# leggedrobotics/delora

Measured on AMD Instinct MI355X. Metric: training scan-pairs/sec, KITTI 64x2048 range images, higher is better.
Workload: dtype f32; 1 GPU; KITTI-shaped 64x2048, batch=8 pairs/GPU, raw scans of ~141k points (ragged, raster order), steps rotate over 8 distinct HBM-resident batches, online normals, ResNet pose CNN (11.9M params, identity-pretrained state), Adam; BASELINE configs[1]; global_batch=8, parallelism=dp1, cnn=fp32, cnn_impl=hip trunk: fp32 MFMA, fused Winograd F(2x2,3x3) + direct implicit GEMM, channels_last=False, hip_graph=False, distinct_batches=8, priming_steps=8

## Files before the change

delora_amd/csrc/conv.hip:

```cpp
#include <type_traits>

#include "common.h"
#include "conv_geom.h"
#include "wgrad_batch.h"

typedef float f32x16 __attribute__((ext_vector_type(16)));
typedef float f32x4 __attribute__((ext_vector_type(4)));

__device__ __forceinline__ __amdgpu_buffer_rsrc_t cv_rsrc(const float* base, unsigned bytes) {
  return __builtin_amdgcn_make_buffer_rsrc(const_cast<float*>(base), 0, (int)bytes, 0x00020000);
}
__device__ __forceinline__ f32x4 cv_ld16(__amdgpu_buffer_rsrc_t rs, unsigned voff, unsigned soff) {
  return __builtin_bit_cast(f32x4, __builtin_amdgcn_raw_buffer_load_b128(rs, (int)voff, (int)soff, 0));
}
#define CV_ZERO_OFF 0x80000000u

#define CV_THREADS 256
#define CV_EPI_ADD 1u
#define CV_EPI_ACT 2u
#define CV_EPI_DACT 4u
#define CV_EPI_ADD_GRID 8u
#define CV_ACT_NONE 0
#define CV_ACT_TANH 1
#define CV_ACT_RELU 2
// ... 4 lines not shown
  float* y;
  const float* add;
  const float* dsrc;
  int N, H, W, C, K, Ho, Wo;
  int act;
  unsigned epi;
  int Hout, Wout;
  int wrap;
  const float* seam;
};

__device__ __forceinline__ float cv_act(float v, int act) {
  if (act == CV_ACT_TANH) return dl_tanh(v);
  if (act == CV_ACT_RELU) return v < 0.f ? 0.f : v;
  return v;
}
__device__ __forceinline__ float cv_dact(float y, int act) {
  if (act == CV_ACT_TANH) return 1.f - y * y;
  if (act == CV_ACT_RELU) return y <= 0.f ? 0.f : 1.f;
  return 1.f;
}

__device__ __forceinline__ int cv_xcd_swizzle(int id, int n) {
  const int q = n / 8, r = n % 8, xcd = id % 8, k = id / 8;
  return (xcd < r ? xcd * (q + 1) : r * (q + 1) + (xcd - r) * q) + k;
}

template <int BM, int BN, int CK, int TW, class G, bool BT, int WGN>
#ifndef CV_MINWAVES
#define CV_MINWAVES 2
#endif
__global__ __launch_bounds__(CV_THREADS, CV_MINWAVES) void k_conv_f32(ConvArgs a) {
  constexpr int TH = BM / TW;
  constexpr int SH = G::ISH, SW = G::ISW;
  constexpr int RH = (TH - 1) * SH + G::EH, RW = (TW - 1) * SW + G::EW;
  constexpr int S = CK + 4;
  constexpr int TAPS = G::NT;
  constexpr int C4 = CK / 4;
  constexpr int IN_FLOATS = RH * RW * S;
  constexpr int W_FLOATS = BT ? TAPS * CK * BN : TAPS * BN * S;
  constexpr int NI = RH * RW * C4;
  constexpr int NW = BT ? CK * TAPS * (BN / 4) : BN * TAPS * C4;
  constexpr int NI_IT = (NI + CV_THREADS - 1) / CV_THREADS, NW_IT = (NW + CV_THREADS - 1) / CV_THREADS;
  constexpr int WGM = 4 / WGN;
  constexpr int WM = BM / 32 / WGM, WN = BN / 32 / WGN;
  static_assert(BM % TW == 0 && BM % (32 * WGM) == 0 && BN % (32 * WGN) == 0 && CK % 8 == 0, "tile shape");
  static_assert(TAPS > 0, "a stride phase without taps has no launch");
  static_assert((S / 4) % 2 == 1, "pixel stride must be 4*odd floats");
  constexpr int EPW = WN * 32, ES = EPW + 4;
  constexpr int LDS_HOLD = (BM == 256 && TW == 128 && CK == 8 && BT) ? 160 * 1024 / 3 / 4 + 16 : 0;
  constexpr int LDS_USED = IN_FLOATS + W_FLOATS > 4 * 32 * ES ? IN_FLOATS + W_FLOATS : 4 * 32 * ES;
  constexpr int LDS_FLOATS = LDS_USED > LDS_HOLD ? LDS_USED : LDS_HOLD;
  __shared__ __attribute__((aligned(16))) float lds[LDS_FLOATS];
  float* in_lds = lds;
  float* w_lds = lds + IN_FLOATS;

  const int tid = threadIdx.x, lane = tid & 63, wave = tid >> 6;
  const int li = lane & 31, half = lane >> 5;
  const int wm = wave / WGN, wn = wave % WGN;
  const int KT = a.K / BN;
  const int tiles_w = (a.Wo + TW - 1) / TW, tiles_h = (a.Ho + TH - 1) / TH;
  const int ntiles = a.N * tiles_h * tiles_w * KT;
  const int t = cv_xcd_swizzle(blockIdx.x, ntiles);
  const int kt = t % KT;
  int pt = t / KT;
  const int tw_i = pt % tiles_w; pt /= tiles_w;
  const int th_i = pt % tiles_h;
  const int n = pt / tiles_h;
  const int ho0 = th_i * TH, wo0 = tw_i * TW, k0 = kt * BN;
  const int h_base = ho0 * SH + G::H0, w_base = wo0 * SW + G::W0;
  const float* xn = a.x + (size_t)n * a.H * a.W * a.C;

  const unsigned x_bytes = (unsigned)(a.H * a.W * a.C) * 4u, w_bytes = (unsigned)(a.K * a.C * G::WTAPS) * 4u;
  const __amdgpu_buffer_rsrc_t x_rs = cv_rsrc(xn, x_bytes), w_rs = cv_rsrc(a.w, w_bytes);
  const unsigned x_zero = CV_ZERO_OFF;
  unsigned in_g[NI_IT];
  int in_l[NI_IT];
#pragma unroll
  for (int it = 0; it < NI_IT; ++it) {
    const int q = min(tid + it * CV_THREADS, NI - 1);
    const int c4 = q % C4, pc = q / C4;
    const int col = pc % RW, row = pc / RW;
    const int h = h_base + row;
    int w = w_base + col;
    const bool col_in = w >= 0 && w < a.W;
    w = w < 0 ? w + a.W : w;
    w = w >= a.W ? w - a.W : w;
    in_l[it] = pc * S + c4 * 4;
    in_g[it] = (h >= 0 && h < a.H && (a.wrap ? w < a.W : col_in)) ? (unsigned)((h * a.W + w) * a.C + c4 * 4) * 4u : x_zero;
  }
  unsigned w_g[NW_IT];
  int w_l[NW_IT];
#pragma unroll
  for (int it = 0; it < NW_IT; ++it) {
    const int q = min(tid + it * CV_THREADS, NW - 1);
    if (!BT) {
      const int c4 = q % C4, t2 = q / C4;
      const int tap = t2 % TAPS, kk = t2 / TAPS;
      w_g[it] = (unsigned)(((k0 + kk) * G::WTAPS + G::wt(tap)) * a.C + c4 * 4) * 4u;
      w_l[it] = (tap * BN + kk) * S + c4 * 4;
    } else {
      const int co4 = q % (BN / 4), t2 = q / (BN / 4);
      const int tap = t2 % TAPS, kr = t2 / TAPS;
      w_g[it] = (unsigned)((kr * G::WTAPS + G::wt(tap)) * a.K + k0 + co4 * 4) * 4u;
      w_l[it] = (tap * CK + kr) * BN + co4 * 4;
    }
  }

  f32x16 acc[WM][WN];
#pragma unroll
  for (int i = 0; i < WM; ++i)
#pragma unroll
    for (int j = 0; j < WN; ++j)
#pragma unroll
      for (int r = 0; r < 16; ++r) acc[i][j][r] = 0.f;

  int a_off[WM];
// ... 371 lines not shown
};
__global__ __launch_bounds__(CV_THREADS) void k_wgrad_reduce_batch(WgReduceBatchArgs b) {
  const int l = dl_table_slot<DL_WGRAD_BATCH>(b.first_block, b.n, (int)blockIdx.x);
  dl_slab_sum_body(b.part[l], b.nslabs[l], b.count[l], b.dw[l], ((size_t)((int)blockIdx.x - b.first_block[l]) * CV_THREADS + threadIdx.x) * 4);
}
__global__ __launch_bounds__(CV_THREADS) void k_wgrad_reduce(const float* __restrict__ part, int nslabs, size_t count,
                                                             float* __restrict__ dw) {
  dl_slab_sum_body(part, nslabs, count, dw, ((size_t)blockIdx.x * CV_THREADS + threadIdx.x) * 4);
}


template <int BM, int BN, int CK, int TW, class G, bool BT, int WGN>
static int launch_conv(const ConvArgs& a, hipStream_t st) {
  constexpr int TH = BM / TW;
  if (a.K % BN || a.C % CK) return 1;
  const int ntiles = a.N * ((a.Ho + TH - 1) / TH) * ((a.Wo + TW - 1) / TW) * (a.K / BN);
  const double px_ = (double)a.N * a.Ho * a.Wo;
  constexpr int ks_ = G::WTAPS == 9 ? 3 : 1;
  const DlProfTag tag{"k_conv_f32", BT ? "dgrad" : "fwd", a.N, a.H, a.W, a.C, a.K, ks_, BT ? G::OSH : G::ISH, BT ? G::OSW : G::ISW, 2.0 * px_ * a.K * a.C * G::NT,
                      4.0 * ((double)a.N * a.H * a.W * a.C + px_ * a.K + (double)G::WTAPS * a.K * a.C)};
  DL_LAUNCH(tag, (k_conv_f32<BM, BN, CK, TW, G, BT, WGN>), dim3(ntiles), dim3(CV_THREADS), st, a);
  return 0;
}

#ifndef CV_BN
#define CV_BN 64
#endif
#ifndef CV_CK
#define CV_CK 16
#endif
#ifndef CV_WGN
#define CV_WGN 2
#endif

#ifdef CV_TUNE
int g_cv_variant = 0;
template <class G, bool BT, int BM, int BN, int CKK, int WGNN>
static int variant_conv(const ConvArgs& a, hipStream_t st) {
  if (a.Wo % 128 == 0 && !launch_conv<BM, BN, CKK, 128, G, BT, WGNN>(a, st)) return 0;
  if (a.Wo % 64 == 0 && !launch_conv<BM, BN, CKK, 64, G, BT, WGNN>(a, st)) return 0;
  return 1;
}
#endif

static int cv_pick_tw(int Ho, int Wo, int bm, int min_tw) {
  int best = 0;
  long best_px = 0;
  for (int tw = 128; tw >= min_tw; tw >>= 1) {
    const int th = bm / tw;
    if (th < 1) continue;
    const long px = (long)((Ho + th - 1) / th) * th * (long)((Wo + tw - 1) / tw) * tw;
    if (!best || px < best_px) { best = tw; best_px = px; }
  }
  return best;
}

template <class G, bool BT, int CKK>
static int launch_conv_128(const ConvArgs& a, hipStream_t st) {
  switch (cv_pick_tw(a.Ho, a.Wo, 128, 16)) {
    case 128: return launch_conv<128, CV_BN, CKK, 128, G, BT, CV_WGN>(a, st);
    case 64: return launch_conv<128, CV_BN, CKK, 64, G, BT, CV_WGN>(a, st);
    case 32: return launch_conv<128, CV_BN, CKK, 32, G, BT, CV_WGN>(a, st);
    default: return launch_conv<128, CV_BN, CKK, 16, G, BT, CV_WGN>(a, st);
  }
}

template <class G, bool BT, bool BIG>
static int dispatch_conv(const ConvArgs& a, hipStream_t st) {
#ifdef CV_TUNE
  if constexpr (BIG) {
    switch (g_cv_variant) {
      case 1: return variant_conv<G, BT, 128, 64, 8, 2>(a, st);
      case 2: return variant_conv<G, BT, 128, 64, 32, 2>(a, st);
      case 3: return variant_conv<G, BT, 128, 128, 8, 2>(a, st);
      case 4: return variant_conv<G, BT, 128, 128, 16, 2>(a, st);
      case 5: return variant_conv<G, BT, 256, 64, 8, 1>(a, st);
      case 6: return variant_conv<G, BT, 256, 64, 16, 1>(a, st);
      case 7: return variant_conv<G, BT, 256, 128, 8, 2>(a, st);
      case 8: return variant_conv<G, BT, 128, 64, 16, 1>(a, st);
      case 9: return variant_conv<G, BT, 256, 128, 16, 2>(a, st);
      default: break;
    }
  }
#endif
  if constexpr (BIG) {
    if (a.C >= 256) {
      if (a.Wo % 128 == 0 && a.Ho % 2 == 0 && !launch_conv<256, 64, 16, 128, G, BT, 1>(a, st)) return 0;
      if (a.Wo % 64 == 0 && a.Ho % 4 == 0 && !launch_conv<256, 64, 16, 64, G, BT, 1>(a, st)) return 0;
    } else {
      if (a.Wo % 128 == 0 && a.Ho % 2 == 0 && !launch_conv<256, 64, 8, 128, G, BT, 1>(a, st)) return 0;
      if (a.Wo % 64 == 0 && a.Ho % 4 == 0 && !launch_conv<256, 64, 8, 64, G, BT, 1>(a, st)) return 0;
    }
  }
  if constexpr (G::WTAPS == 9 && !BIG && !BT && G::ISH == 1 && G::ISW == 2) {
    if (a.C <= 256 && a.Wo % 128 == 0 && a.Ho % 2 == 0 && !launch_conv<256, 64, 8, 128, G, BT, 1>(a, st)) return 0;
  }
  if constexpr (G::WTAPS == 9 && !BIG) {
    if (a.C % CV_CK || a.C <= 256) return launch_conv_128<G, BT, 8>(a, st);
  }
  return launch_conv_128<G, BT, CV_CK>(a, st);
}

#define FX_ROWS 16
#define FX_KMAX 512
__global__ __launch_bounds__(CV_THREADS) void k_dgrad_oddw_seam(const float* __restrict__ g, const float* __restrict__ w, float* __restrict__ seam,
                                                                int N, int Ho, int Wo, int K, int C, int H, int SH) {
  constexpr int GROWS = FX_ROWS + 2;
  __shared__ float gs[(GROWS + 1) * FX_KMAX];
  const int side = blockIdx.y;
  const int row_tiles = (H + FX_ROWS - 1) / FX_ROWS;
  const int n = blockIdx.x / row_tiles, h0 = (blockIdx.x % row_tiles) * FX_ROWS;
  const int lane = threadIdx.x & 63, wave = threadIdx.x >> 6;
  const int c = blockIdx.z * 64 + lane, cc = c < C ? c : C - 1;
  const int s = side ? 0 : 2, wo = side ? 0 : Wo - 1;
  const int ho_lo = h0 > 0 ? (h0 - 1) / SH : 0;
  int src[FX_ROWS][3];
#pragma unroll
  for (int i = 0; i < FX_ROWS; ++i)
#pragma unroll
    for (int r = 0; r < 3; ++r) {
      const int t = h0 + i + 1 - r;
      const int ho = t / SH;
      const bool ok = t >= 0 && t % SH == 0 && ho < Ho && ho - ho_lo >= 0 && ho - ho_lo < GROWS;
      src[i][r] = (ok ? ho - ho_lo : GROWS) * FX_KMAX;
    }
  float acc[FX_ROWS];
#pragma unroll
  for (int i = 0; i < FX_ROWS; ++i) acc[i] = 0.f;
  for (int k0 = 0; k0 < K; k0 += FX_KMAX) {
    const int kn = K - k0 < FX_KMAX ? K - k0 : FX_KMAX;
    __syncthreads();
// ... 261 lines not shown
```

delora_amd/csrc/wino.hip:

```cpp
#include "common.h"
#include "wgrad_batch.h"
#include <cstdlib>

typedef float f32x16 __attribute__((ext_vector_type(16)));
typedef float f32x4 __attribute__((ext_vector_type(4)));
typedef float f32x2 __attribute__((ext_vector_type(2)));
typedef int i32x4 __attribute__((ext_vector_type(4)));

#define WN_THREADS 512
#define WN_CK 8
#define WN_KB 64
#define WN_TILES 64
#define WN_PLANE (WN_TILES * WN_CK + 16)
#define WN_EPI_ADD 1u
#define WN_EPI_ACT 2u
#define WN_EPI_DACT 4u

struct WinoArgs {
  const float* x;
  const float* u;
  float* y;
  const float* add;
  const float* dsrc;
  int N, H, W, C, K;
// ... 125 lines not shown
#define WN_IF_U(...)
#else
#define WN_IF_U(...) __VA_ARGS__
#endif
#if WN_ABL & 2
#define WN_IF_RAW(...)
#else
#define WN_IF_RAW(...) __VA_ARGS__
#endif
#if WN_ABL & 4
#define WN_IF_T(...)
#else
#define WN_IF_T(...) __VA_ARGS__
#endif
#if WN_ABL & 8
#define WN_IF_BAR(...)
#else
#define WN_IF_BAR(...) __VA_ARGS__
#endif
#if WN_ABL & 16
#define WN_IF_FR(...)
#else
#define WN_IF_FR(...) __VA_ARGS__
#endif
#ifdef CV_TUNE
__device__ unsigned long long g_wn_t[8 * 8192];
#define WN_T(I) { if (tid == 0 && grp < 8192) g_wn_t[grp * 8 + (I)] = clock64(); }
#else
#define WN_T(I)
#endif
template <int TC, bool RAG, bool SPLIT = false>
__global__ __launch_bounds__(WN_THREADS) void k_wino_conv(WinoArgs a) {
  constexpr int STR = 0;
#include "wino_conv_body.h"
}
template <int TC, int STR>
__global__ __launch_bounds__(WN_THREADS) void k_wino_conv_strided(WinoArgs a) {
  constexpr bool RAG = false, SPLIT = false;
#include "wino_conv_body.h"
}

struct WinoBatchArgs {
  const float* w[DL_WINO_BATCH];
  float* u_fwd[DL_WINO_BATCH];
  float* u_bwd[DL_WINO_BATCH];
  int K[DL_WINO_BATCH], C[DL_WINO_BATCH];
  int first_block[DL_WINO_BATCH + 1];
  int n;
};
__global__ __launch_bounds__(256) void k_wino_weights_batch(WinoBatchArgs a) {
  __shared__ float stage[16 * 256];
  const int l = dl_table_slot<DL_WINO_BATCH>(a.first_block, a.n, (int)blockIdx.x);
  const int K = a.K[l], C = a.C[l];
  const int blk = (int)blockIdx.x - a.first_block[l];
  const int cblocks = C / 32;
  const int k0 = (blk / cblocks) * 8, c0 = (blk % cblocks) * 32;
  if (k0 >= K) return;
  const float* __restrict__ w = a.w[l];
  float* __restrict__ u_fwd = a.u_fwd[l];
  float* __restrict__ u_bwd = a.u_bwd[l];
  const int t = threadIdx.x, kk = t >> 5, cc = t & 31;
  const int k = k0 + kk, c = c0 + cc;
  float g[3][3], gf[3][3], u[4][4];
#pragma unroll
  for (int r = 0; r < 3; ++r)
#pragma unroll
    for (int s2 = 0; s2 < 3; ++s2) {
      g[r][s2] = w[((size_t)(k * 3 + r) * 3 + s2) * C + c];
      gf[2 - r][2 - s2] = g[r][s2];
// ... 1188 lines not shown

static bool wn_strided_tiles(int N, int H, int W, int C, int K, int sh, int sw, int* tc) {
  if (sh != 1 || sw != 2 || N <= 0 || H <= 0 || W <= 0 || C <= 0 || K <= 0 || (H & 1) || (W & 3) || C % 64 || K % 64) return false;
  const int wide = 2 * C > K ? 2 * C : K;
  if ((size_t)N * H * (W / 2) * wide >= ((size_t)1 << 31) || (size_t)H * (W / 2) * wide >= ((size_t)1 << 30)) return false;
  const int tw = W / 4, th = H / 2;
  if (tw % 32 == 0 && th % 2 == 0) { *tc = 32; return true; }
  if (tw % 16 == 0 && th % 4 == 0) { *tc = 16; return true; }
  return false;
}

extern "C" int dl_wino_strided_takes(int32_t N, int32_t H, int32_t W, int32_t C, int32_t K, int32_t stride_h, int32_t stride_w,
                                     int32_t cu_count) {
  int tc;
  if (!wn_strided_tiles(N, H, W, C, K, stride_h, stride_w, &tc)) return 0;
  const int cap = cu_count > 0 ? cu_count : wn_cu_count();
  return wino_plan(N, H, W / 2, 2 * C, K, cap).splits == 1 && wino_plan(N, H, W / 2, K, 2 * C, cap).splits == 1;
}

extern "C" size_t dl_wino_strided_weights_floats(int32_t K, int32_t C, int32_t stride_h, int32_t stride_w) {
  return stride_h == 1 && stride_w == 2 && K > 0 && C > 0 ? (size_t)16 * K * 2 * C : 0;
}

extern "C" int dl_wino_strided_weights_f32(const float* w, float* u_fwd, float* u_bwd, int32_t K, int32_t C, int32_t stride_h,
                                           int32_t stride_w, dl_stream stream) {
  if (!w || (!u_fwd && !u_bwd) || K <= 0 || C <= 0 || K % 8 || C % 8 || stride_h != 1 || stride_w != 2)
    return dl_fail(DL_ERR_INVALID_ARGUMENT, "dl_wino_strided_weights_f32: bad argument (K, C multiples of 8, stride (1,2))");
  hipLaunchKernelGGL(k_wino_weights_strided, dim3((K * 2 * C + 255) / 256), dim3(256), 0, (hipStream_t)stream, w, u_fwd, u_bwd, K, C);
  return dl_check_launch("dl_wino_strided_weights_f32");
}

static int wn_strided_launch(const char* what, WinoArgs a, int str, int tc, int H, int W, int C, int K, int sh, int sw, hipStream_t st) {
  const int tw = a.W / 2, th = a.H / 2;
  const DlProfTag tag{"k_wino_conv", "conv", a.N, H, W, C, K, 3, sh, sw, 2.0 * 12.0 * (double)a.N * th * tw * (double)a.C * a.K,
                      4.0 * ((double)a.N * a.H * a.W * (a.C + a.K) + 12.0 * a.C * a.K)};
  const int groups = a.N * (th / (WN_TILES / tc)) * (tw / tc) * (a.K / WN_KB);
  const int cap = wn_cu_count();
  const dim3 grid(cap > 0 && groups > cap ? cap : groups);
  if (str == 1) {
    if (tc == 32) DL_LAUNCH(tag, (k_wino_conv_strided<32, 1>), grid, dim3(WN_THREADS), st, a);
    else DL_LAUNCH(tag, (k_wino_conv_strided<16, 1>), grid, dim3(WN_THREADS), st, a);
  } else {
    if (tc == 32) DL_LAUNCH(tag, (k_wino_conv_strided<32, 2>), grid, dim3(WN_THREADS), st, a);
    else DL_LAUNCH(tag, (k_wino_conv_strided<16, 2>), grid, dim3(WN_THREADS), st, a);
  }
  return dl_check_launch(what);
}

extern "C" int dl_wino_strided_conv3x3_nhwc_f32(const float* x, const float* u_fwd, float* y, int32_t N, int32_t H, int32_t W, int32_t C,
                                                int32_t K, int32_t stride_h, int32_t stride_w, int32_t act, uint32_t epilogue,
                                                dl_stream stream) {
  if (!x || !u_fwd || !y || act < 0 || act > 2 || (epilogue & ~WN_EPI_ACT))
    return dl_fail(DL_ERR_INVALID_ARGUMENT, "dl_wino_strided_conv3x3_nhwc_f32: bad argument (epilogue: the activation bit or none)");
  int tc;
  if (!wn_strided_tiles(N, H, W, C, K, stride_h, stride_w, &tc))
    return dl_fail(DL_ERR_UNSUPPORTED, "dl_wino_strided_conv3x3_nhwc_f32: N=%d H=%d W=%d C=%d K=%d stride (%d,%d) does not tile", N, H, W, C, K, stride_h, stride_w);
  WinoArgs a{x, u_fwd, y, nullptr, nullptr, N, H, W / 2, 2 * C, K, act, epilogue, 1};
  return wn_strided_launch("dl_wino_strided_conv3x3_nhwc_f32", a, 1, tc, H, W, C, K, stride_h, stride_w, (hipStream_t)stream);
}

extern "C" int dl_wino_strided_dgrad3x3_nhwc_f32(const float* g, const float* u_bwd, float* dx, const float* add_grid, const float* dsrc,
                                                 int32_t N, int32_t H, int32_t W, int32_t K, int32_t C, int32_t stride_h, int32_t stride_w,
                                                 int32_t act, uint32_t epilogue, dl_stream stream) {
  const uint32_t EPI_GRID = 8u;
  if (!g || !u_bwd || !dx || act < 0 || act > 2 || (epilogue & ~(EPI_GRID | WN_EPI_DACT)) || ((epilogue & EPI_GRID) && !add_grid) ||
      ((epilogue & WN_EPI_DACT) && !dsrc))
    return dl_fail(DL_ERR_INVALID_ARGUMENT, "dl_wino_strided_dgrad3x3_nhwc_f32: bad argument (epilogue bits 8 / 4 and their operands)");
  int tc;
  if (!wn_strided_tiles(N, H, W, C, K, stride_h, stride_w, &tc))
    return dl_fail(DL_ERR_UNSUPPORTED, "dl_wino_strided_dgrad3x3_nhwc_f32: N=%d H=%d W=%d C=%d K=%d stride (%d,%d) does not tile", N, H, W, C, K, stride_h, stride_w);
  const unsigned epi = ((epilogue & EPI_GRID) ? WN_EPI_ADD : 0u) | (epilogue & WN_EPI_DACT);
  WinoArgs a{g, u_bwd, dx, add_grid, dsrc, N, H, W / 2, K, 2 * C, act, epi, 1};
  return wn_strided_launch("dl_wino_strided_dgrad3x3_nhwc_f32", a, 2, tc, H, W, C, K, stride_h, stride_w, (hipStream_t)stream);
}
```

delora_amd/csrc/wino_conv_body.h:

```cpp
  constexpr int DEAD = STR == 1 ? 3 : (STR == 2 ? 0 : -1);
  constexpr int TR = WN_TILES / TC;
  constexpr int RH = 2 * TR + 2, RW = 2 * TC + 2;
  constexpr int NPIX = RH * RW, NRI = (NPIX + 31) / 32;
  constexpr int RAWBUF = NRI * 256;
  constexpr int NR_IT = (NRI + 7) / 8;
  constexpr int BUF = 2 * 16 * WN_PLANE;
  static_assert((2 * BUF + 2 * RAWBUF) * 4 <= 163840, "LDS budget");
  __shared__ __attribute__((aligned(16))) float lds[2 * BUF + 2 * RAWBUF];
  float* rawbase = lds + 2 * BUF;
#define WN_BUFOF(CH) (lds + (((CH) + 1) & 1) * BUF)

  const int tid = threadIdx.x, lane = tid & 63, wave = __builtin_amdgcn_readfirstlane(tid >> 6);
  const int li = lane & 31, half = lane >> 5;
  const int mb = wave & 1, nb = (wave >> 1) & 1, xh = wave >> 2;
  const int KT = a.K / WN_KB;
  const int tiles_w = RAG ? ((a.W + 1) / 2 + TC - 1) / TC : (a.W / 2) / TC;
  const int tiles_h = RAG ? ((a.H + 1) / 2 + TR - 1) / TR : (a.H / 2) / TR;
  const int nsplit = SPLIT ? a.splits : 1;
  const int ngroups = a.N * tiles_h * tiles_w * KT * nsplit;
  const int nchunks = a.C / WN_CK / nsplit;

  const int tb = wave & 3, tc4 = lane & 1, ttile = (wave >> 2) * 32 + (lane >> 1);
  const int ttr = ttile / TC, ttc = ttile % TC;
  const int j0 = tb == 0 ? 0 : (tb == 2 ? 2 : 1), j1 = tb == 2 ? 1 : (tb == 3 ? 3 : 2);
  const float sgn_s = tb == 1 ? 1.f : -1.f;
  const f32x2 sgn = {sgn_s, sgn_s};
  const int t_wr = tb * WN_PLANE + ttile * 8 + ((tc4 ^ ((ttile >> 3) & 1)) * 4);
  const int t_rd = ((2 * ttr) * RW + 2 * ttc) * 8 + tc4 * 4;
  constexpr int NRAW_W = (NRI + 1) / 2;
  const unsigned lane16 = 16u * (unsigned)lane;
  const int arow = mb * 32 + li, brow = nb * 32 + li;
  const int a_off = arow * 8 + ((half ^ ((arow >> 3) & 1)) * 4);
  const int b_off = 16 * WN_PLANE + brow * 8 + ((half ^ ((brow >> 3) & 1)) * 4);

  int n, k0, gh, gw;
  int cb = 0;
  float* ysp = a.y;
  const float* xn;
  int rowmask[4];
  bool edge;
  unsigned raw_g[NR_IT];
#define WN_SETUP(G, LN)                                                                                                   \
  {                                                                                                                       \
    int t_ = wn_xcd_swizzle((G), ngroups);                                                                                \
    if (SPLIT) { cb = (t_ % nsplit) * nchunks; t_ /= nsplit; }        \
    const int kt_ = t_ % KT; t_ /= KT;                                                                                    \
    gw = t_ % tiles_w; t_ /= tiles_w;                                                                                     \
    gh = t_ % tiles_h;                                                                                                    \
    n = t_ / tiles_h;                                                                                                     \
    k0 = kt_ * WN_KB;                                                                                                     \
    const int h_base_ = gh * TR * 2 - 1, w_base_ = gw * TC * 2 - 1;                       \
    xn = a.x + (size_t)n * a.H * a.W * a.C;                                                                               \
    _Pragma("unroll") for (int i = 0; i < 4; ++i) {                                                                       \
      const int h_ = h_base_ + 2 * ttr + i;                                                                               \
      rowmask[i] = (h_ >= 0 && h_ < a.H) ? -1 : 0;                                                                        \
    }                                                                                                                     \
    edge = __builtin_amdgcn_readfirstlane((int)(h_base_ < 0 || h_base_ + RH > a.H)) != 0;                                                                           \
    _Pragma("unroll") for (int it = 0; it < NR_IT; ++it) {                                                                \
      const int p_ = min(min(2 * wave + it, NRI - 1) * 32 + ((LN) >> 1), NPIX - 1);         \
      int h_ = h_base_ + p_ / RW;                                                                                         \
      h_ = h_ < 0 ? 0 : (h_ >= a.H ? a.H - 1 : h_);                                                                       \
      int w_ = w_base_ + p_ % RW;                                                                                         \
      if (RAG) { w_ %= a.W; w_ = w_ < 0 ? w_ + a.W : w_; }        \
      else w_ = w_ < 0 ? w_ + a.W : (w_ >= a.W ? w_ - a.W : w_);                                                           \
      raw_g[it] = 4u * (unsigned)((h_ * a.W + w_) * a.C + ((LN) & 1) * 4);                                       \
    }                                                                                                                     \
  }

  const unsigned lds_base = (unsigned)(__SIZE_TYPE__)((__attribute__((address_space(3))) char*)lds);
  const int m0_raw = __builtin_amdgcn_readfirstlane((int)(lds_base + 4u * (unsigned)(2 * BUF + min(2 * wave, NRI - 1) * 256)));
  const int m0_u = __builtin_amdgcn_readfirstlane((int)(lds_base + 4u * (unsigned)(16 * WN_PLANE + 2 * wave * WN_PLANE)));
#define WN_RAW_ALL(CH)                                                                                                    \
  {                                                                                                                       \
    const float* rp_ = xn + ((CH) + cb) * WN_CK;                                                                          \
    const int m_ = m0_raw + ((CH) & 1) * (RAWBUF * 4);                                                                    \
    if (2 * wave + 1 < NRI)                                                                                               \
      asm volatile("s_mov_b32 m0, %0\n\ts_nop 0\n\tglobal_load_lds_dwordx4 %1, %3\n\tglobal_load_lds_dwordx4 %2, %4 offset:1024"     \
                   :: "s"(m_), "v"(raw_g[0]), "v"(raw_g[NR_IT - 1]), "s"(rp_), "s"(rp_ - 256) : "memory");                  \
    else if (2 * wave < NRI)                                                                                              \
      asm volatile("s_mov_b32 m0, %0\n\ts_nop 0\n\tglobal_load_lds_dwordx4 %1, %2" :: "s"(m_), "v"(raw_g[0]), "s"(rp_) : "memory");  \
  }
#define WN_U_ALL(CH, BUFP)                                                                                                \
  {                                                                                                                       \
    const float* up_ = a.u + (((size_t)((CH) + cb) * KT + (k0 >> 6)) * 16 + 2 * wave) * 512;                               \
    const int m_ = m0_u + (int)((BUFP) - lds) * 4;                                                                        \
    if (DEAD == 3 && (wave & 1))                                                 \
      asm volatile("s_mov_b32 m0, %0\n\ts_nop 0\n\tglobal_load_lds_dwordx4 %1, %2\n\tglobal_load_lds_dwordx4 %1, %2 offset:1024" \
                   :: "s"(m_), "v"(lane16), "s"(up_) : "memory");                                                         \
    else if (DEAD == 0 && !(wave & 1))                                                           \
      asm volatile("s_mov_b32 m0, %0\n\ts_nop 0\n\tglobal_load_lds_dwordx4 %1, %2 offset:2112\n\tglobal_load_lds_dwordx4 %1, %2 offset:3136" \
                   :: "s"(m_), "v"(lane16), "s"(up_ - 16) : "memory");                                                    \
    else                                                                                                                  \
    asm volatile("s_mov_b32 m0, %0\n\ts_nop 0\n\tglobal_load_lds_dwordx4 %1, %2\n\tglobal_load_lds_dwordx4 %1, %2 offset:1024\n\t" \
                 "global_load_lds_dwordx4 %1, %3 offset:2112\n\tglobal_load_lds_dwordx4 %1, %3 offset:3136"                \
                 :: "s"(m_), "v"(lane16), "s"(up_), "s"(up_ - 16) : "memory");                                            \
  }
#define WN_TROW_LD(I, RB)                                                                                                 \
  {                                                                                                                       \
    dd[(I) & 1][0] = *reinterpret_cast<const i32x4*>((RB) + t_rd + ((I) * RW + j0) * 8);                                  \
    dd[(I) & 1][1] = *reinterpret_cast<const i32x4*>((RB) + t_rd + ((I) * RW + j1) * 8);                                  \
  }
#define WN_TROW_FIN(I)                                                                                                    \
  {                                                                                                                       \
    if (edge) { asm volatile("" ::: "memory"); dd[(I) & 1][0] &= rowmask[I]; dd[(I) & 1][1] &= rowmask[I]; }      \
    const f32x4 da_ = __builtin_bit_cast(f32x4, dd[(I) & 1][0]), db_ = __builtin_bit_cast(f32x4, dd[(I) & 1][1]);         \
    asm volatile("v_pk_fma_f32 %0, %1, %2, %3" : "=v"(tt[I][0]) : "v"(__builtin_shufflevector(db_, db_, 0, 1)), "s"(sgn), "v"(__builtin_shufflevector(da_, da_, 0, 1))); \
    asm volatile("v_pk_fma_f32 %0, %1, %2, %3" : "=v"(tt[I][1]) : "v"(__builtin_shufflevector(db_, db_, 2, 3)), "s"(sgn), "v"(__builtin_shufflevector(da_, da_, 2, 3))); \
  }
#define WN_TROW(I, RB) WN_TROW_LD(I, RB) WN_TROW_FIN(I)
#define WN_PK_ADD(X, Y) ({ f32x2 l_, h_;                                                                                    \
    asm volatile("v_pk_add_f32 %0, %1, %2" : "=v"(l_) : "v"((X)[0]), "v"((Y)[0]));                                        \
    asm volatile("v_pk_add_f32 %0, %1, %2" : "=v"(h_) : "v"((X)[1]), "v"((Y)[1]));                                        \
    __builtin_shufflevector(l_, h_, 0, 1, 2, 3); })
#define WN_PK_SUB(X, Y) ({ f32x2 l_, h_;                                                                                    \
    asm volatile("v_pk_add_f32 %0, %1, %2 neg_lo:[0,1] neg_hi:[0,1]" : "=v"(l_) : "v"((X)[0]), "v"((Y)[0]));              \
    asm volatile("v_pk_add_f32 %0, %1, %2 neg_lo:[0,1] neg_hi:[0,1]" : "=v"(h_) : "v"((X)[1]), "v"((Y)[1]));              \
    __builtin_shufflevector(l_, h_, 0, 1, 2, 3); })
#define WN_V0()                                                                                                           \
  {                                                                                                                       \
    f32x2 tt[4][2];                                                                                                       \
    i32x4 dd[2][2];                                                                                                       \
    const float* rb_ = rawbase;                                                                                           \
    float* vb_ = WN_BUFOF(0) + t_wr;                                                                                      \
    WN_TROW(0, rb_) WN_TROW(1, rb_) WN_TROW(2, rb_) WN_TROW(3, rb_)                                                       \
    *reinterpret_cast<f32x4*>(vb_ + 0 * 4 * WN_PLANE) = WN_PK_SUB(tt[0], tt[2]);                                                    \
    *reinterpret_cast<f32x4*>(vb_ + 1 * 4 * WN_PLANE) = WN_PK_ADD(tt[1], tt[2]);                                                    \
    *reinterpret_cast<f32x4*>(vb_ + 2 * 4 * WN_PLANE) = WN_PK_SUB(tt[2], tt[1]);                                                    \
    *reinterpret_cast<f32x4*>(vb_ + 3 * 4 * WN_PLANE) = WN_PK_SUB(tt[1], tt[3]);                                                    \
  }
// ... 8 lines not shown
    acc[XL] = __builtin_amdgcn_mfma_f32_32x32x2f32(av[(XL) & 1][J], bv[(XL) & 1][J], acc[XL], 0, 0, 0);                   \
    __VA_ARGS__                                                                                                           \
    __builtin_amdgcn_sched_barrier(0);                                                                                    \
  }
#define WN_MZ(XL, J, ...)                                                                                                 \
  {                                                                                                                       \
    acc[XL] = __builtin_amdgcn_mfma_f32_32x32x2f32(av[(XL) & 1][J], bv[(XL) & 1][J], wn_zero16, 0, 0, 0);                 \
    __VA_ARGS__                                                                                                           \
    __builtin_amdgcn_sched_barrier(0);                                                                                    \
  }
#define WN_LOAD_FRAGS_B(XL, B, BP)                                                                                        \
  {                                                                                                                       \
    av[B] = *reinterpret_cast<const f32x4*>((BP) + (xh * 8 + (XL)) * WN_PLANE + a_off);                                   \
    bv[B] = *reinterpret_cast<const f32x4*>((BP) + (xh * 8 + (XL)) * WN_PLANE + b_off);                                   \
  }
#define WN_MB(XL, B, J, ...)                                                                                              \
  {                                                                                                                       \
    acc[XL] = __builtin_amdgcn_mfma_f32_32x32x2f32(av[B][J], bv[B][J], acc[XL], 0, 0, 0);                                 \
    __VA_ARGS__                                                                                                           \
    __builtin_amdgcn_sched_barrier(0);                                                                                    \
  }
#define WN_MZB(XL, B, J, ...)                                                                                             \
  {                                                                                                                       \
    acc[XL] = __builtin_amdgcn_mfma_f32_32x32x2f32(av[B][J], bv[B][J], wn_zero16, 0, 0, 0);                               \
    __VA_ARGS__                                                                                                           \
    __builtin_amdgcn_sched_barrier(0);                                                                                    \
  }

  const f32x16 wn_zero16 = {0.f, 0.f, 0.f, 0.f, 0.f, 0.f, 0.f, 0.f, 0.f, 0.f, 0.f, 0.f, 0.f, 0.f, 0.f, 0.f};
  int grp = blockIdx.x;
  WN_SETUP(grp, lane)
  WN_RAW_ALL(0)
  WN_RAW_ALL(min(1, nchunks - 1))
  WN_U_ALL(0, WN_BUFOF(0))
  asm volatile("s_waitcnt vmcnt(0)" ::: "memory");
  __syncthreads();
  WN_V0()
  for (;;) {
    __syncthreads();
    WN_T(0)
    f32x4 av[2], bv[2];
    f32x2 tt[4][2];
    i32x4 dd[2][2];
    f32x16 acc[8];
    {
      float* cur = WN_BUFOF(0);
      if (DEAD == 0) WN_LOAD_FRAGS_B(1, 0, cur)
      else WN_LOAD_FRAGS(0)
    }
#define WN_CHUNK_BODY(MF)                                                                                                 \
    {                                                                                                                     \
      float* cur = WN_BUFOF(ch);                                                                                          \
      float* nxt = WN_BUFOF(ch + 1);                                                                                      \
      const float* rb = rawbase + ((ch + 1) & 1) * RAWBUF;                                                                \
      float* vb = nxt + t_wr;                                                                                             \
      MF(0, 0, WN_IF_FR(WN_LOAD_FRAGS(1))) WN_M(0, 1, WN_IF_U(WN_U_ALL(ch + 1, nxt)))                                     \
      WN_M(0, 2, )                                                                                                        \
                            \
      WN_M(0, 3, WN_IF_RAW(if (ch + 2 < nchunks) WN_RAW_ALL(ch + 2)))                                                     \
       \
      MF(1, 0, WN_IF_FR(WN_LOAD_FRAGS(2))) WN_M(1, 1, WN_IF_T(WN_TROW_LD(0, rb) WN_TROW_LD(1, rb))) WN_M(1, 2, ) WN_M(1, 3, WN_IF_T(WN_TROW_FIN(0) WN_TROW_FIN(1))) \
      MF(2, 0, WN_IF_FR(WN_LOAD_FRAGS(3))) WN_M(2, 1, WN_IF_T(WN_TROW_LD(2, rb) WN_TROW_LD(3, rb))) WN_M(2, 2, ) WN_M(2, 3, WN_IF_T(WN_TROW_FIN(2) WN_TROW_FIN(3))) \
      MF(3, 0, WN_IF_FR(WN_LOAD_FRAGS(4)) WN_IF_T(*reinterpret_cast<f32x4*>(vb + 0 * 4 * WN_PLANE) = WN_PK_SUB(tt[0], tt[2]);))   \
      WN_M(3, 1, WN_IF_T(*reinterpret_cast<f32x4*>(vb + 1 * 4 * WN_PLANE) = WN_PK_ADD(tt[1], tt[2]);)) WN_M(3, 2, ) WN_M(3, 3, ) \
      MF(4, 0, WN_IF_FR(WN_LOAD_FRAGS(5)) WN_IF_T(*reinterpret_cast<f32x4*>(vb + 2 * 4 * WN_PLANE) = WN_PK_SUB(tt[2], tt[1]);))   \
      WN_M(4, 1, WN_IF_T(*reinterpret_cast<f32x4*>(vb + 3 * 4 * WN_PLANE) = WN_PK_SUB(tt[1], tt[3]);)) WN_M(4, 2, ) WN_M(4, 3, ) \
      MF(5, 0, WN_IF_FR(WN_LOAD_FRAGS(6))) WN_M(5, 1, ) WN_M(5, 2, ) WN_M(5, 3, )                                         \
      MF(6, 0, WN_IF_FR(WN_LOAD_FRAGS(7))) WN_M(6, 1, ) WN_M(6, 2, ) WN_M(6, 3, )                                         \
      asm volatile("s_waitcnt vmcnt(0) lgkmcnt(0)" ::: "memory");                                                         \
      WN_IF_BAR(__builtin_amdgcn_s_barrier();)                                                                            \
      __builtin_amdgcn_sched_barrier(0);                                                                                  \
      MF(7, 0, WN_IF_FR(WN_LOAD_FRAGS_FROM(0, nxt))) WN_M(7, 1, ) WN_M(7, 2, ) WN_M(7, 3, )                               \
    }
#define WN_TAIL_BODY(MF)                                                                                                  \
    {                                                                                                                     \
      float* cur = WN_BUFOF(nchunks - 1);                                                                                 \
      MF(0, 0, WN_LOAD_FRAGS(1)) WN_M(0, 1, ) WN_M(0, 2, ) WN_M(0, 3, )                                                   \
      MF(1, 0, WN_LOAD_FRAGS(2)) WN_M(1, 1, ) WN_M(1, 2, ) WN_M(1, 3, )                                                   \
      MF(2, 0, WN_LOAD_FRAGS(3)) WN_M(2, 1, ) WN_M(2, 2, ) WN_M(2, 3, )                                                   \
      MF(3, 0, WN_LOAD_FRAGS(4)) WN_M(3, 1, ) WN_M(3, 2, ) WN_M(3, 3, )                                                   \
// ... 36 lines not shown
      MF(6, 1, 0, ) WN_MB(6, 1, 1, ) WN_MB(6, 1, 2, ) WN_MB(6, 1, 3, )                                                    \
    }
#define WN_CHUNK_BODY_B(MF)                                                                                               \
    {                                                                                                                     \
      float* cur = WN_BUFOF(ch);                                                                                          \
      float* nxt = WN_BUFOF(ch + 1);                                                                                      \
      const float* rb = rawbase + ((ch + 1) & 1) * RAWBUF;                                                                \
      float* vb = nxt + t_wr;                                                                                             \
      MF(1, 0, 0, WN_LOAD_FRAGS_B(2, 1, cur) WN_U_ALL(ch + 1, nxt))                                                       \
      WN_MB(1, 0, 1, WN_TX(WN_TROW_LD(0, rb) WN_TROW_LD(1, rb)))                                                          \
      WN_MB(1, 0, 2, if (ch + 2 < nchunks) WN_RAW_ALL(ch + 2)) WN_MB(1, 0, 3, WN_TX(WN_TROW_FIN(0) WN_TROW_FIN(1)))       \
      MF(2, 1, 0, WN_LOAD_FRAGS_B(3, 0, cur)) WN_MB(2, 1, 1, WN_TX(WN_TROW_LD(2, rb) WN_TROW_LD(3, rb))) WN_MB(2, 1, 2, ) \
      WN_MB(2, 1, 3, WN_TX(WN_TROW_FIN(2) WN_TROW_FIN(3)))                                                                \
      MF(3, 0, 0, WN_LOAD_FRAGS_B(5, 1, cur) WN_VST(0, WN_PK_SUB(tt[0], tt[2])))                                          \
      WN_MB(3, 0, 1, WN_VST(1, WN_PK_ADD(tt[1], tt[2]))) WN_MB(3, 0, 2, ) WN_MB(3, 0, 3, )                                \
      MF(5, 1, 0, WN_LOAD_FRAGS_B(6, 0, cur) WN_VST(2, WN_PK_SUB(tt[2], tt[1])))                                          \
      WN_MB(5, 1, 1, WN_VST(3, WN_PK_SUB(tt[1], tt[3]))) WN_MB(5, 1, 2, ) WN_MB(5, 1, 3, )                                \
      MF(6, 0, 0, WN_LOAD_FRAGS_B(7, 1, cur)) WN_MB(6, 0, 1, ) WN_MB(6, 0, 2, ) WN_MB(6, 0, 3, )                          \
      asm volatile("s_waitcnt vmcnt(0) lgkmcnt(0)" ::: "memory");                                                         \
      __builtin_amdgcn_s_barrier();                                                                                       \
      __builtin_amdgcn_sched_barrier(0);                                                                                  \
      MF(7, 1, 0, WN_LOAD_FRAGS_B(1, 0, nxt)) WN_MB(7, 1, 1, ) WN_MB(7, 1, 2, ) WN_MB(7, 1, 3, )                          \
    }
#define WN_TAIL_BODY_B(MF)                                                                                                \
    {                                                                                                                     \
      float* cur = WN_BUFOF(nchunks - 1);                                                                                 \
      MF(1, 0, 0, WN_LOAD_FRAGS_B(2, 1, cur)) WN_MB(1, 0, 1, ) WN_MB(1, 0, 2, ) WN_MB(1, 0, 3, )                          \
      MF(2, 1, 0, WN_LOAD_FRAGS_B(3, 0, cur)) WN_MB(2, 1, 1, ) WN_MB(2, 1, 2, ) WN_MB(2, 1, 3, )                          \
      MF(3, 0, 0, WN_LOAD_FRAGS_B(5, 1, cur)) WN_MB(3, 0, 1, ) WN_MB(3, 0, 2, ) WN_MB(3, 0, 3, )                          \
      MF(5, 1, 0, WN_LOAD_FRAGS_B(6, 0, cur)) WN_MB(5, 1, 1, ) WN_MB(5, 1, 2, ) WN_MB(5, 1, 3, )                          \
      MF(6, 0, 0, WN_LOAD_FRAGS_B(7, 1, cur)) WN_MB(6, 0, 1, ) WN_MB(6, 0, 2, ) WN_MB(6, 0, 3, )                          \
      MF(7, 1, 0, ) WN_MB(7, 1, 1, ) WN_MB(7, 1, 2, ) WN_MB(7, 1, 3, )                                                    \
    }
    if (DEAD == 3) {
      if (nchunks > 1) {
        { const int ch = 0; WN_CHUNK_BODY_F(WN_MZB) }
        for (int ch = 1; ch + 1 < nchunks; ++ch) WN_CHUNK_BODY_F(WN_MB)
        WN_TAIL_BODY_F(WN_MB)
      } else WN_TAIL_BODY_F(WN_MZB)
    } else if (DEAD == 0) {
      if (nchunks > 1) {
        { const int ch = 0; WN_CHUNK_BODY_B(WN_MZB) }
        for (int ch = 1; ch + 1 < nchunks; ++ch) WN_CHUNK_BODY_B(WN_MB)
        WN_TAIL_BODY_B(WN_MB)
      } else WN_TAIL_BODY_B(WN_MZB)
    } else
    if (nchunks > 1) {
      { const int ch = 0; WN_CHUNK_BODY(WN_MZ) }
      for (int ch = 1; ch + 1 < nchunks; ++ch) WN_CHUNK_BODY(WN_M)
      WN_TAIL_BODY(WN_M)
    } else WN_TAIL_BODY(WN_MZ)
#undef WN_CHUNK_BODY
#undef WN_TAIL_BODY
#undef WN_CHUNK_BODY_F
#undef WN_TAIL_BODY_F
#undef WN_CHUNK_BODY_B
#undef WN_TAIL_BODY_B
#undef WN_TX
#undef WN_VST
    __syncthreads();
    WN_T(1)

    int lane_e = lane;
    asm volatile("" : "+v"(lane_e));
    const int li_e = lane_e & 31, half_e = lane_e >> 5;
    unsigned ooff[8];
    {
      const int lcol = (lane_e >> 4) * 2 + ((lane_e >> 3) & 1);
      const unsigned lane_off = (unsigned)(lcol * a.K + (lane_e & 7) * 4);
#pragma unroll
      for (int it = 0; it < 8; ++it) {
        const int ut = 4 * (mb * 8 + it), tr = ut / TC, tc = ut % TC;
        const int oh = (gh * TR + tr) * 2 + xh, ow0 = (gw * TC + tc) * 2;
        ooff[it] = (unsigned)(((n * a.H + oh) * a.W + ow0) * a.K + k0 + nb * 32) + lane_off;
        if (RAG && (oh >= a.H || ow0 + lcol >= a.W)) ooff[it] = 0xffffffffu;
      }
    }
    unsigned goff[8];
    bool grid_block = true;
    if (STR == 2) {
      const int kh = a.K >> 1;
      const int lcol = (lane_e >> 4) * 2 + ((lane_e >> 3) & 1);
      grid_block = k0 < kh;
#pragma unroll
      for (int it = 0; it < 8; ++it) {
        const int ut = 4 * (mb * 8 + it), tr = ut / TC, tc = ut % TC;
        const int oh = (gh * TR + tr) * 2 + xh, ow0 = (gw * TC + tc) * 2;
        goff[it] = grid_block ? (unsigned)(((n * a.H + oh) * a.W + ow0 + lcol) * kh + k0 + nb * 32 + (lane_e & 7) * 4) : 0u;
      }
    }
    const unsigned (&aoff)[8] = STR == 2 ? goff : ooff;
    if (SPLIT) ysp = a.y + (size_t)(cb / nchunks) * ((size_t)a.N * a.H * a.W * a.K);
    const int nextg = grp + gridDim.x;
    const bool more = nextg < ngroups;
    if (more) {
      WN_SETUP(nextg, lane_e)
      WN_RAW_ALL(0)
      WN_RAW_ALL(min(1, nchunks - 1))
      WN_U_ALL(0, WN_BUFOF(0))
    }

    f32x16 keep[2];
    float* xch = lds;
    const int blk = wave & 3;
    {
      float* dst = xch + ((blk * 2 + xh) * 32) * 64 + lane_e;
#pragma unroll
      for (int q = 0; q < 2; ++q) {
        f32x16 p0, p1;
        if (DEAD == 0) {
          if (q == 0) { p0 = acc[1] + acc[2]; p1 = acc[5] + acc[6]; }
          else        { p0 = wn_sub16(wn_sub16(acc[1], acc[2]), acc[3]); p1 = wn_sub16(wn_sub16(acc[5], acc[6]), acc[7]); }
        } else if (DEAD == 3) {
          if (q == 0) { p0 = acc[0] + acc[1] + acc[2]; p1 = acc[4] + acc[5] + acc[6]; }
          else        { p0 = wn_sub16(acc[1], acc[2]); p1 = wn_sub16(acc[5], acc[6]); }
        } else
        if (q == 0) { p0 = acc[0] + acc[1] + acc[2]; p1 = acc[4] + acc[5] + acc[6]; }
        else        { p0 = wn_sub16(wn_sub16(acc[1], acc[2]), acc[3]); p1 = wn_sub16(wn_sub16(acc[5], acc[6]), acc[7]); }
        f32x16 snd;
        if (xh == 0) { keep[q] = p0 + p1; snd = p1; }
        else         { keep[q] = wn_nsub16(p0, p1); snd = p0; }
#pragma unroll
        for (int r = 0; r < 16; ++r) dst[(q * 16 + r) * 64] = snd[r];
        __builtin_amdgcn_sched_barrier(0);
      }
    }
    const bool f_add = (a.epi & WN_EPI_ADD) && (STR != 2 || grid_block), f_act = a.epi & WN_EPI_ACT, f_dact = a.epi & WN_EPI_DACT;
    __syncthreads();
    {
      const float* src = xch + ((blk * 2 + (xh ^ 1)) * 32) * 64 + lane_e;
#pragma unroll
      for (int q = 0; q < 2; ++q)
// ... 25 lines not shown
    WN_T(3)
    const bool tanh_act = a.act == 1;
    if (tanh_act || !(f_act || f_dact)) {
      const float* epl = ep + (lane_e >> 3) * ES + (lane_e & 7) * 4;
      if (f_dact) { if (f_add) wn_store_items<true, false, true, RAG>(epl, opv, ooff, aoff, ysp, a.add); else wn_store_items<false, false, true, RAG>(epl, opv, ooff, aoff, ysp, a.add); }
      else if (f_act) { if (f_add) wn_store_items<true, true, false, RAG>(epl, opv, ooff, aoff, ysp, a.add); else wn_store_items<false, true, false, RAG>(epl, opv, ooff, aoff, ysp, a.add); }
      else { if (f_add) wn_store_items<true, false, false, RAG>(epl, opv, ooff, aoff, ysp, a.add); else wn_store_items<false, false, false, RAG>(epl, opv, ooff, aoff, ysp, a.add); }
    } else
#pragma unroll
    for (int it = 0; it < 8; ++it) {
      const int i = lane_e + it * 64, row = i >> 3, c4 = i & 7;
      if (RAG && ooff[it] == 0xffffffffu) continue;
      f32x4 v = *reinterpret_cast<const f32x4*>(ep + row * ES + c4 * 4);
      if (f_add) v += f_dact ? *reinterpret_cast<const f32x4*>(a.add + aoff[it]) : opv[it];
      if (f_act) {
        if (tanh_act) { v[0] = dl_tanh(v[0]); v[1] = dl_tanh(v[1]); v[2] = dl_tanh(v[2]); v[3] = dl_tanh(v[3]); }
        else { v[0] = wn_act(v[0], a.act); v[1] = wn_act(v[1], a.act); v[2] = wn_act(v[2], a.act); v[3] = wn_act(v[3], a.act); }
      }
      if (f_dact) {
        const f32x4 sv = opv[it];
        if (tanh_act) v *= 1.f - sv * sv;
        else { v[0] *= wn_dact(sv[0], a.act); v[1] *= wn_dact(sv[1], a.act); v[2] *= wn_dact(sv[2], a.act); v[3] *= wn_dact(sv[3], a.act); }
      }
      *reinterpret_cast<f32x4*>(ysp + ooff[it]) = v;
    }
    WN_T(4)
    if (!more) break;
    grp = nextg;
  }
#undef WN_BUFOF
#undef WN_SETUP
#undef WN_RAW_ALL
#undef WN_U_ALL
#undef WN_TROW
#undef WN_PK_ADD
#undef WN_PK_SUB
#undef WN_TROW_LD
#undef WN_TROW_FIN
#undef WN_V0
#undef WN_LOAD_FRAGS
#undef WN_LOAD_FRAGS_FROM
#undef WN_M
#undef WN_MZ
#undef WN_LOAD_FRAGS_B
#undef WN_MB
#undef WN_MZB
```

Baseline: 696.5 scan-pairs/s.

## Skip dead Winograd planes in strided convs and compact 1x1 strided conv loads

Adds a phase-aware (PH) path to the strided Winograd kernel that computes only 8 of the 12 transform planes for output channels whose grid/phase makes the rest zero. It also rotates K-tile assignment across XCDs to balance the lighter and heavier blocks. Separately, 1x1 strided direct convs now load a compact input tile, sampling every stride-th pixel instead of the full strided span, and use a dedicated CK. This removes MFMA and LDS work in stride-2 convs, at the cost of more complex macro code and an env fallback to the old path.

Measured after the change: 702.1 scan-pairs/s (median of 6 runs). No clear change (+0.8%).

```diff
diff --git a/delora_amd/csrc/conv.hip b/delora_amd/csrc/conv.hip
--- a/delora_amd/csrc/conv.hip
+++ b/delora_amd/csrc/conv.hip
@@ -60,7 +60,9 @@
 #endif
 __global__ __launch_bounds__(CV_THREADS, CV_MINWAVES) void k_conv_f32(ConvArgs a) {
   constexpr int TH = BM / TW;
-  constexpr int SH = G::ISH, SW = G::ISW;
+  constexpr bool COMPACT = G::EH == 1 && G::EW == 1;
+  constexpr int GH = COMPACT ? G::ISH : 1, GW = COMPACT ? G::ISW : 1;
+  constexpr int SH = COMPACT ? 1 : G::ISH, SW = COMPACT ? 1 : G::ISW;
   constexpr int RH = (TH - 1) * SH + G::EH, RW = (TW - 1) * SW + G::EW;
   constexpr int S = CK + 4;
   constexpr int TAPS = G::NT;
@@ -96,7 +98,7 @@
   const int th_i = pt % tiles_h;
   const int n = pt / tiles_h;
   const int ho0 = th_i * TH, wo0 = tw_i * TW, k0 = kt * BN;
-  const int h_base = ho0 * SH + G::H0, w_base = wo0 * SW + G::W0;
+  const int h_base = ho0 * G::ISH + G::H0, w_base = wo0 * G::ISW + G::W0;
   const float* xn = a.x + (size_t)n * a.H * a.W * a.C;
 
   const unsigned x_bytes = (unsigned)(a.H * a.W * a.C) * 4u, w_bytes = (unsigned)(a.K * a.C * G::WTAPS) * 4u;
@@ -109,8 +111,8 @@
     const int q = min(tid + it * CV_THREADS, NI - 1);
     const int c4 = q % C4, pc = q / C4;
     const int col = pc % RW, row = pc / RW;
-    const int h = h_base + row;
-    int w = w_base + col;
+    const int h = h_base + row * GH;
+    int w = w_base + col * GW;
     const bool col_in = w >= 0 && w < a.W;
     w = w < 0 ? w + a.W : w;
     w = w >= a.W ? w - a.W : w;
@@ -548,6 +550,9 @@
 #ifndef CV_WGN
 #define CV_WGN 2
 #endif
+#ifndef CV_CK_1X1S
+#define CV_CK_1X1S 16
+#endif
 
 #ifdef CV_TUNE
 int g_cv_variant = 0;
@@ -613,6 +618,9 @@
   }
   if constexpr (G::WTAPS == 9 && !BIG) {
     if (a.C % CV_CK || a.C <= 256) return launch_conv_128<G, BT, 8>(a, st);
+  }
+  if constexpr (G::WTAPS == 1 && !BT && (G::ISH > 1 || G::ISW > 1)) {
+    if (a.C % CV_CK_1X1S == 0) return launch_conv_128<G, BT, CV_CK_1X1S>(a, st);
   }
   return launch_conv_128<G, BT, CV_CK>(a, st);
 }
diff --git a/delora_amd/csrc/wino.hip b/delora_amd/csrc/wino.hip
--- a/delora_amd/csrc/wino.hip
+++ b/delora_amd/csrc/wino.hip
@@ -181,9 +181,10 @@
 template <int TC, bool RAG, bool SPLIT = false>
 __global__ __launch_bounds__(WN_THREADS) void k_wino_conv(WinoArgs a) {
   constexpr int STR = 0;
+  constexpr bool PH = false;
 #include "wino_conv_body.h"
 }
-template <int TC, int STR>
+template <int TC, int STR, bool PH>
 __global__ __launch_bounds__(WN_THREADS) void k_wino_conv_strided(WinoArgs a) {
   constexpr bool RAG = false, SPLIT = false;
 #include "wino_conv_body.h"
@@ -1438,17 +1439,27 @@
 
 static int wn_strided_launch(const char* what, WinoArgs a, int str, int tc, int H, int W, int C, int K, int sh, int sw, hipStream_t st) {
   const int tw = a.W / 2, th = a.H / 2;
-  const DlProfTag tag{"k_wino_conv", "conv", a.N, H, W, C, K, 3, sh, sw, 2.0 * 12.0 * (double)a.N * th * tw * (double)a.C * a.K,
-                      4.0 * ((double)a.N * a.H * a.W * (a.C + a.K) + 12.0 * a.C * a.K)};
+  static const bool all12 = [] { const char* e = getenv("DL_WINO_STRIDED_ALL12"); return e && e[0] == '1'; }();
+  const double planes = all12 ? 12.0 : 10.0;
+  const DlProfTag tag{"k_wino_conv", "conv", a.N, H, W, C, K, 3, sh, sw, 2.0 * planes * (double)a.N * th * tw * (double)a.C * a.K,
+                      4.0 * ((double)a.N * a.H * a.W * (a.C + a.K) + planes * a.C * a.K)};
   const int groups = a.N * (th / (WN_TILES / tc)) * (tw / tc) * (a.K / WN_KB);
   const int cap = wn_cu_count();
   const dim3 grid(cap > 0 && groups > cap ? cap : groups);
-  if (str == 1) {
-    if (tc == 32) DL_LAUNCH(tag, (k_wino_conv_strided<32, 1>), grid, dim3(WN_THREADS), st, a);
-    else DL_LAUNCH(tag, (k_wino_conv_strided<16, 1>), grid, dim3(WN_THREADS), st, a);
+  if (all12) {
+    if (str == 1) {
+      if (tc == 32) DL_LAUNCH(tag, (k_wino_conv_strided<32, 1, false>), grid, dim3(WN_THREADS), st, a);
+      else DL_LAUNCH(tag, (k_wino_conv_strided<16, 1, false>), grid, dim3(WN_THREADS), st, a);
+    } else {
+      if (tc == 32) DL_LAUNCH(tag, (k_wino_conv_strided<32, 2, false>), grid, dim3(WN_THREADS), st, a);
+      else DL_LAUNCH(tag, (k_wino_conv_strided<16, 2, false>), grid, dim3(WN_THREADS), st, a);
+    }
+  } else if (str == 1) {
+    if (tc == 32) DL_LAUNCH(tag, (k_wino_conv_strided<32, 1, true>), grid, dim3(WN_THREADS), st, a);
+    else DL_LAUNCH(tag, (k_wino_conv_strided<16, 1, true>), grid, dim3(WN_THREADS), st, a);
   } else {
-    if (tc == 32) DL_LAUNCH(tag, (k_wino_conv_strided<32, 2>), grid, dim3(WN_THREADS), st, a);
-    else DL_LAUNCH(tag, (k_wino_conv_strided<16, 2>), grid, dim3(WN_THREADS), st, a);
+    if (tc == 32) DL_LAUNCH(tag, (k_wino_conv_strided<32, 2, true>), grid, dim3(WN_THREADS), st, a);
+    else DL_LAUNCH(tag, (k_wino_conv_strided<16, 2, true>), grid, dim3(WN_THREADS), st, a);
   }
   return dl_check_launch(what);
 }
diff --git a/delora_amd/csrc/wino_conv_body.h b/delora_amd/csrc/wino_conv_body.h
--- a/delora_amd/csrc/wino_conv_body.h
+++ b/delora_amd/csrc/wino_conv_body.h
@@ -40,11 +40,13 @@
   int rowmask[4];
   bool edge;
   unsigned raw_g[NR_IT];
-#define WN_SETUP(G, LN)                                                                                                   \
+  const int ph_d = STR == 2 && PH ? max(1, (int)gridDim.x / 8 / KT) : 1;
+#define WN_SETUP(G, LN)                                                                                                  \
   {                                                                                                                       \
     int t_ = wn_xcd_swizzle((G), ngroups);                                                                                \
     if (SPLIT) { cb = (t_ % nsplit) * nchunks; t_ /= nsplit; }        \
-    const int kt_ = t_ % KT; t_ /= KT;                                                                                    \
+    int kt_ = t_ % KT; t_ /= KT;                                                                                          \
+    if (STR == 2 && PH) kt_ = (kt_ + (t_ / ph_d) * (KT >> 1)) % KT;        \
     gw = t_ % tiles_w; t_ /= tiles_w;                                                                                     \
     gh = t_ % tiles_h;                                                                                                    \
     n = t_ / tiles_h;                                                                                                     \
@@ -95,6 +97,22 @@
                  "global_load_lds_dwordx4 %1, %3 offset:2112\n\tglobal_load_lds_dwordx4 %1, %3 offset:3136"                \
                  :: "s"(m_), "v"(lane16), "s"(up_), "s"(up_ - 16) : "memory");                                            \
   }
+#define WN_U_ALL8(CH, BUFP)                                                                                               \
+  {                                                                                                                       \
+    const float* up_ = a.u + (((size_t)((CH) + cb) * KT + (k0 >> 6)) * 16 + 2 * wave) * 512;                               \
+    const int m_ = m0_u + (int)((BUFP) - lds) * 4;                                                                        \
+    if (wave & 1)                                                                                                         \
+      asm volatile("s_mov_b32 m0, %0\n\ts_nop 0\n\tglobal_load_lds_dwordx4 %1, %2\n\tglobal_load_lds_dwordx4 %1, %2 offset:1024" \
+                   :: "s"(m_), "v"(lane16), "s"(up_) : "memory");                                                         \
+    else                                                                                                                  \
+      asm volatile("s_mov_b32 m0, %0\n\ts_nop 0\n\tglobal_load_lds_dwordx4 %1, %2 offset:2112\n\tglobal_load_lds_dwordx4 %1, %2 offset:3136" \
+                   :: "s"(m_), "v"(lane16), "s"(up_ - 16) : "memory");                                                    \
+  }
+#define WN_U_FIRST()                                                                                                      \
+  {                                                                                                                       \
+    if (PH && (STR == 1 || k0 < (a.K >> 1))) WN_U_ALL8(0, WN_BUFOF(0))                                                    \
+    else WN_U_ALL(0, WN_BUFOF(0))                                                                                         \
+  }
 #define WN_TROW_LD(I, RB)                                                                                                 \
   {                                                                                                                       \
     dd[(I) & 1][0] = *reinterpret_cast<const i32x4*>((RB) + t_rd + ((I) * RW + j0) * 8);                                  \
@@ -169,7 +187,7 @@
   WN_SETUP(grp, lane)
   WN_RAW_ALL(0)
   WN_RAW_ALL(min(1, nchunks - 1))
-  WN_U_ALL(0, WN_BUFOF(0))
+  WN_U_FIRST()
   asm volatile("s_waitcnt vmcnt(0)" ::: "memory");
   __syncthreads();
   WN_V0()
@@ -182,7 +200,7 @@
     f32x16 acc[8];
     {
       float* cur = WN_BUFOF(0);
-      if (DEAD == 0) WN_LOAD_FRAGS_B(1, 0, cur)
+      if (DEAD == 0 || PH) WN_LOAD_FRAGS_B(1, 0, cur)
       else WN_LOAD_FRAGS(0)
     }
 #define WN_CHUNK_BODY(MF)                                                                                                 \
@@ -285,6 +303,57 @@
       MF(6, 0, 0, WN_LOAD_FRAGS_B(7, 1, cur)) WN_MB(6, 0, 1, ) WN_MB(6, 0, 2, ) WN_MB(6, 0, 3, )                          \
       MF(7, 1, 0, ) WN_MB(7, 1, 1, ) WN_MB(7, 1, 2, ) WN_MB(7, 1, 3, )                                                    \
     }
+#define WN_CHUNK_BODY_8(MF, NX0, UALL)                                                                                    \
+    {                                                                                                                     \
+      float* cur = WN_BUFOF(ch);                                                                                          \
+      float* nxt = WN_BUFOF(ch + 1);                                                                                      \
+      const float* rb = rawbase + ((ch + 1) & 1) * RAWBUF;                                                                \
+      float* vb = nxt + t_wr;                                                                                             \
+      MF(1, 0, 0, WN_LOAD_FRAGS_B(2, 1, cur) UALL(ch + 1, nxt))                                                           \
+      WN_MB(1, 0, 1, WN_TX(WN_TROW_LD(0, rb) WN_TROW_LD(1, rb)))                                                          \
+      WN_MB(1, 0, 2, if (ch + 2 < nchunks) WN_RAW_ALL(ch + 2)) WN_MB(1, 0, 3, WN_TX(WN_TROW_FIN(0) WN_TROW_FIN(1)))       \
+      MF(2, 1, 0, WN_LOAD_FRAGS_B(5, 0, cur)) WN_MB(2, 1, 1, WN_TX(WN_TROW_LD(2, rb) WN_TROW_LD(3, rb))) WN_MB(2, 1, 2, ) \
+      WN_MB(2, 1, 3, WN_TX(WN_TROW_FIN(2) WN_TROW_FIN(3)))                                                                \
+      MF(5, 0, 0, WN_LOAD_FRAGS_B(6, 1, cur) WN_VST(0, WN_PK_SUB(tt[0], tt[2])))                                          \
+      WN_MB(5, 0, 1, WN_VST(1, WN_PK_ADD(tt[1], tt[2])) WN_VST(2, WN_PK_SUB(tt[2], tt[1])))                               \
+      WN_MB(5, 0, 2, WN_VST(3, WN_PK_SUB(tt[1], tt[3]))) WN_MB(5, 0, 3, )                                                 \
+      asm volatile("s_waitcnt vmcnt(0) lgkmcnt(0)" ::: "memory");                                                         \
+      __builtin_amdgcn_s_barrier();                                                                                       \
+      __builtin_amdgcn_sched_barrier(0);                                                                                  \
+      MF(6, 1, 0, WN_LOAD_FRAGS_B(NX0, 0, nxt)) WN_MB(6, 1, 1, ) WN_MB(6, 1, 2, ) WN_MB(6, 1, 3, )                        \
+    }
+#define WN_TAIL_BODY_8(MF)                                                                                                \
+    {                                                                                                                     \
+      float* cur = WN_BUFOF(nchunks - 1);                                                                                 \
+      MF(1, 0, 0, WN_LOAD_FRAGS_B(2, 1, cur)) WN_MB(1, 0, 1, ) WN_MB(1, 0, 2, ) WN_MB(1, 0, 3, )                          \
+      MF(2, 1, 0, WN_LOAD_FRAGS_B(5, 0, cur)) WN_MB(2, 1, 1, ) WN_MB(2, 1, 2, ) WN_MB(2, 1, 3, )                          \
+      MF(5, 0, 0, WN_LOAD_FRAGS_B(6, 1, cur)) WN_MB(5, 0, 1, ) WN_MB(5, 0, 2, ) WN_MB(5, 0, 3, )                          \
+      MF(6, 1, 0, ) WN_MB(6, 1, 1, ) WN_MB(6, 1, 2, ) WN_MB(6, 1, 3, )                                                    \
+    }
+#define WN_MB_SEAM(XL, B, J, ...) WN_SEAM_PICK(XL)(XL, B, J, __VA_ARGS__)
+#define WN_SEAM_PICK(XL) WN_SEAM_##XL
+#define WN_SEAM_0 WN_MZB
+#define WN_SEAM_4 WN_MZB
+#define WN_SEAM_1 WN_MB
+#define WN_SEAM_2 WN_MB
+#define WN_SEAM_5 WN_MB
+#define WN_SEAM_6 WN_MB
+    if (DEAD == 3 && PH) {
+      const int nev = nchunks >> 1;
+      { const int ch = 0; WN_CHUNK_BODY_8(WN_MZB, 1, WN_U_ALL8) }
+      for (int ch = 1; ch + 1 < nev; ++ch) WN_CHUNK_BODY_8(WN_MB, 1, WN_U_ALL8)
+      { const int ch = nev - 1; WN_CHUNK_BODY_8(WN_MB, 0, WN_U_ALL) }
+      { const int ch = nev; WN_CHUNK_BODY_F(WN_MB_SEAM) }
+      for (int ch = nev + 1; ch + 1 < nchunks; ++ch) WN_CHUNK_BODY_F(WN_MB)
+      WN_TAIL_BODY_F(WN_MB)
+    } else if (DEAD == 0 && PH && k0 < (a.K >> 1)) {
+      if (nchunks > 1) {
+        { const int ch = 0; WN_CHUNK_BODY_8(WN_MZB, 1, WN_U_ALL8) }
+        for (int ch = 1; ch + 1 < nchunks; ++ch) WN_CHUNK_BODY_8(WN_MB, 1, WN_U_ALL8)
+        WN_TAIL_BODY_8(WN_MB)
+      } else WN_TAIL_BODY_8(WN_MZB)
+      acc[3] = wn_zero16; acc[7] = wn_zero16;
+    } else
     if (DEAD == 3) {
       if (nchunks > 1) {
         { const int ch = 0; WN_CHUNK_BODY_F(WN_MZB) }
@@ -309,6 +378,16 @@
 #undef WN_TAIL_BODY_F
 #undef WN_CHUNK_BODY_B
 #undef WN_TAIL_BODY_B
+#undef WN_CHUNK_BODY_8
+#undef WN_TAIL_BODY_8
+#undef WN_MB_SEAM
+#undef WN_SEAM_PICK
+#undef WN_SEAM_0
+#undef WN_SEAM_4
+#undef WN_SEAM_1
+#undef WN_SEAM_2
+#undef WN_SEAM_5
+#undef WN_SEAM_6
 #undef WN_TX
 #undef WN_VST
     __syncthreads();
@@ -350,7 +429,7 @@
       WN_SETUP(nextg, lane_e)
       WN_RAW_ALL(0)
       WN_RAW_ALL(min(1, nchunks - 1))
-      WN_U_ALL(0, WN_BUFOF(0))
+      WN_U_FIRST()
     }
 
     f32x16 keep[2];
@@ -442,6 +521,8 @@
 #undef WN_SETUP
 #undef WN_RAW_ALL
 #undef WN_U_ALL
+#undef WN_U_ALL8
+#undef WN_U_FIRST
 #undef WN_TROW
 #undef WN_PK_ADD
 #undef WN_PK_SUB
```
